# XiangpengHao/pq-vector

Measured on AMD Instinct MI355X. Metric: topk_queries_per_s_k10, higher is better.
Workload: dtype f32

## Files before the change

### pq-vector_amd/csrc/api.cpp

```cpp
#include "../../include/pqv.h"

#include <hip/hip_runtime.h>
#include <time.h>
#include <unistd.h>

#include <algorithm>
#include <atomic>
#include <functional>
#include <system_error>
#include <thread>
#include <cmath>
#include <chrono>
#include <cstdio>
#include <cstdlib>
#include <cstring>
#include <condition_variable>
#include <memory>
#include <mutex>
#include <new>
#include <string>
#include <type_traits>
#include <unordered_map>
#include <unordered_set>
#include <vector>
// ... 344 lines not shown
    mutable bool i8_residual = true;
    mutable DevBuf d_center, d_list_scale, d_list_half, d_list_radius;
    mutable DevBuf d_row_n2i, d_row_res;
    struct Opts {
        int rerank_mode = 0;
        int tile_filter = 1;
        int filter_variant = 0;
        uint32_t cand_cap = 0;
        int screen_f16 = 1;
        int screen_i8 = 1;
        uint32_t seed_rows = 0;
        uint32_t wide_rows = 0;
        uint32_t tile_rows = 0;
        int running_thr = 1;
        int defer = 1;
        int quad_xcd = -1;
        int single_bucket = 1;
        int seed_refine = 1;
        int item_grid = 1;
        int chunk_major = 1;
        int wide_waves = 0;
        int probe_rows = 1;
        int probe_screen = 1;
        uint32_t quad_width = 0;
        uint32_t min_blocks = 0;
        int pair_prune = 1;
        int i8_form = 0;
        int xcd_items = 1;
        int pf96 = 1;
        int drain_min = 0;
        int fork_wide = 0;
        int wide_quads = 1;
        uint32_t wide_quad_rows = 0;
        int list_once = 0;
    };
    mutable Opts opt;
    uint32_t n_files = 0;
    std::vector<uint32_t> seg_off;
    std::vector<uint64_t> row_base;
    uint32_t seg_max_kc = 0;
    bool rr_cap = false;
    DevBuf d_seg_off, d_seg_off64;
    mutable pqv_counters_t counters{};
    mutable bool timing = false;
    mutable std::vector<hipEvent_t> ev;
    mutable std::unique_ptr<pqv_corpus> cos_corpus;
// ... 2574 lines not shown
namespace {

void opts_from_env(pqv_searcher::Opts &o) {
    auto num = [](const char *name, long long dflt) { const char *e = std::getenv(name); return e && *e ? std::strtoll(e, nullptr, 10) : dflt; };
    if (const char *m = std::getenv("PQV_RERANK_MODE")) o.rerank_mode = !std::strcmp(m, "stream") ? 1 : !std::strcmp(m, "tile") ? 2 : 0;
    o.tile_filter = static_cast<int>(std::min<long long>(2, std::max<long long>(0, num("PQV_TILE_FILTER", o.tile_filter))));
    o.filter_variant = static_cast<int>(num("PQV_FILTER_VARIANT", o.filter_variant));
    o.cand_cap = static_cast<uint32_t>(std::max<long long>(0, num("PQV_CAND_CAP", o.cand_cap)));
    o.screen_f16 = num("PQV_SCREEN_F16", o.screen_f16) != 0;
    o.screen_i8 = static_cast<int>(num("PQV_SCREEN_I8", o.screen_i8));
    o.seed_rows = static_cast<uint32_t>(num("PQV_SEED_ROWS", o.seed_rows));
    o.wide_rows = static_cast<uint32_t>(num("PQV_WIDE_ROWS", o.wide_rows));
    o.tile_rows = static_cast<uint32_t>(num("PQV_TILE_ROWS", o.tile_rows));
    o.running_thr = num("PQV_RUNNING_THR", o.running_thr) != 0;
    o.defer = static_cast<int>(num("PQV_DEFER", o.defer));
    o.quad_xcd = static_cast<int>(num("PQV_QUAD_XCD", o.quad_xcd));
    o.wide_waves = static_cast<int>(num("PQV_WIDE_WAVES", o.wide_waves));
    o.item_grid = static_cast<int>(num("PQV_ITEM_GRID", o.item_grid));
    o.chunk_major = static_cast<int>(num("PQV_CHUNK_MAJOR", o.chunk_major));
    o.seed_refine = static_cast<int>(num("PQV_SEED_REFINE", o.seed_refine));
    o.single_bucket = static_cast<int>(num("PQV_SINGLE_BUCKET", o.single_bucket));
    o.probe_rows = static_cast<int>(num("PQV_PROBE_ROWS", o.probe_rows));
    o.probe_screen = static_cast<int>(num("PQV_PROBE_SCREEN", o.probe_screen));
    o.quad_width = static_cast<uint32_t>(num("PQV_QUAD_WIDTH", o.quad_width));
    o.min_blocks = static_cast<uint32_t>(num("PQV_MIN_BLOCKS", o.min_blocks));
    o.wide_quads = static_cast<int>(num("PQV_WIDE_QUADS", o.wide_quads));
    o.fork_wide = static_cast<int>(num("PQV_FORK_WIDE", o.fork_wide));
    o.drain_min = static_cast<int>(num("PQV_DRAIN_MIN", o.drain_min));
    o.pf96 = static_cast<int>(num("PQV_PF96", o.pf96));
    o.xcd_items = static_cast<int>(num("PQV_XCD_ITEMS", o.xcd_items));
    o.wide_quad_rows = static_cast<uint32_t>(num("PQV_WIDE_QUAD_ROWS", o.wide_quad_rows));
    o.list_once = static_cast<int>(num("PQV_LIST_ONCE", o.list_once));
    o.pair_prune = static_cast<int>(num("PQV_PAIR_PRUNE", o.pair_prune));
    o.i8_form = static_cast<int>(num("PQV_I8_FORM", o.i8_form));
}

bool wide_rows_nt(const pqv_searcher *s) {
    if (!s->h_wide_stats.p) return true;
    const volatile uint32_t *h = s->h_wide_stats.as<uint32_t>();
    const uint32_t total = h[0], lone = h[1];
    return total == 0 || static_cast<uint64_t>(lone) * 4 >= static_cast<uint64_t>(total) * 3;
}

bool prefer_regular(const pqv_searcher *s) {
    if (!s->h_wide_stats.p) return false;
    const volatile uint32_t *h = s->h_wide_stats.as<uint32_t>();
// ... 547 lines not shown
    end.assign(clusters.size(), 0);
    uint64_t fb = 0;
    j = 0;
    for (uint32_t f = 0; f < F; ++f) {
        const uint32_t kf = std::min<uint32_t>(nprobe, s->seg_off[f + 1] - s->seg_off[f]);
        for (uint32_t i = 0; i < kf && j < clusters.size(); ++i, ++j) end[j] = fb + quota[f];
        fb += cnt[f];
    }
}

void stream_split(uint64_t max_len, uint64_t pairs, uint32_t &rows_per_block, uint32_t &blocks_per_list) {
    const uint64_t bpl = std::max<uint64_t>(1, std::min<uint64_t>((8192 + pairs - 1) / pairs, (max_len + 255) / 256));
    const uint64_t rpb = ((max_len + bpl - 1) / bpl + 255) / 256 * 256;
    rows_per_block = static_cast<uint32_t>(rpb);
    blocks_per_list = static_cast<uint32_t>((max_len + rpb - 1) / rpb);
}

struct TopkPlan {
    uint32_t np;
    uint32_t probe_bpl;
    uint32_t probe_kpart;
    bool probe_rows;
    bool probe_screen;
    uint32_t rr_rows_per_block, rr_bpl;
    uint32_t n_part_probe, n_part_rr;
    bool tile;
    uint32_t max_groups;
    bool filter;
    uint32_t seed_rows, filter_bpl;
    bool f16;
    bool i8;
    bool quad;
    uint32_t filter_rows_per_block, max_quads, quad_width;
    uint32_t block_waves;
    uint32_t slots_per_pair;
    uint32_t wide_width;
    uint32_t wide_rows_per_block, wide_bpl;
    bool list_once;
};

static uint32_t cand_cap_for(const pqv_searcher *s, uint32_t k) {
    return std::max<uint32_t>(s->opt.cand_cap ? s->opt.cand_cap : (k > 32 ? 8192u : 2048u), k);
}
static bool defer_on(const pqv_searcher *s, uint32_t nq, uint32_t k, const TopkPlan &p) {
    if (s->opt.defer == 0) return false;
    if (k > 64) return true;
    const uint64_t mean_len = s->n / std::max<uint32_t>(1, s->n_clusters);
    if (s->opt.defer != 2 && mean_len > 1536 && prefer_regular(s)) return false;
    return nq >= 8 && p.i8 && p.block_waves == 4 && p.quad_width == 96 && s->sdim >= 512 && (s->opt.defer == 2 || mean_len <= 3072);
}
static bool defer_route(const pqv_searcher *s, uint32_t nq, uint32_t k, const TopkPlan &p) {
    return defer_on(s, nq, k, p) && cand_cap_for(s, k) <= 8192;
}
static bool seed_refine_on(const pqv_searcher *s, uint32_t nq, uint32_t k) {
    (void)nq;
    return s->opt.seed_refine && (!s->d_row_of || s->images_only) && (s->sdim % 32) == 0 && k <= 16 && (s->opt.seed_refine > 1 || s->sdim >= 256);
}
TopkPlan plan_topk(const pqv_searcher *s, uint32_t nq, uint32_t nprobe, uint32_t k = 1, int metric = 0, bool exact_stream = false) {
    TopkPlan p{};
    const pqv_searcher::Opts &o = s->opt;
    if (metric == PQV_DOT) exact_stream = true;
    p.np = probe_count(s, nprobe);
    p.probe_bpl = (s->n_clusters + 255) / 256;
    p.n_part_probe = p.probe_bpl * pqv::waves_per_block();
    p.probe_rows = s->opt.probe_rows && s->kc_pad != 0 && (nq >= 8 || s->opt.probe_rows > 1) &&
                   static_cast<uint64_t>(nq) * s->kc_pad * 12 <= (2ull << 30);
    if (metric == PQV_DOT) p.probe_rows = false;
    p.probe_screen = p.probe_rows && s->ps.ok && o.probe_screen && !s->n_files && p.np >= 1 && p.np <= s->n_clusters / 4 &&
                     (o.probe_screen > 1 || (nq >= 128 && s->n_clusters >= 256));
    p.probe_kpart = p.probe_rows ? 64u : p.np;
    if (s->n_files && !p.probe_rows) {
        p.probe_bpl = (s->seg_max_kc + 255) / 256;
        p.n_part_probe = s->n_files * p.probe_bpl * pqv::waves_per_block();
        p.probe_kpart = std::min<uint32_t>(nprobe, s->seg_max_kc);
    }
    const uint64_t max_len = std::max<uint64_t>(1, s->max_list_len);
    const uint64_t pairs = std::max<uint64_t>(1, static_cast<uint64_t>(nq) * p.np);
    p.tile = metric == PQV_L2SQ_REF4 && k <= 256 && pairs >= 4ull * s->n_clusters;
    const uint64_t mean_len = s->n / std::max<uint32_t>(1, s->n_clusters);
    const bool wide_ok = o.filter_variant == 0 && wide_path_possible(s);
    const bool wide_any_batch = metric == PQV_L2SQ_REF4 && o.tile_filter && k <= 128 && wide_ok && mean_len >= 192;
    if (wide_any_batch) p.tile = true;
    if (o.rerank_mode == 1) p.tile = false;
    if (o.rerank_mode == 2) p.tile = metric == PQV_L2SQ_REF4 && k <= 256;
    if (exact_stream) p.tile = false;
    if (p.tile) {
        const uint64_t est_groups = std::max<uint64_t>(1, pairs / pqv::TILE_QB);
        const uint64_t tile_rows = o.tile_rows ? o.tile_rows : 1536;
        uint64_t rpb = std::min<uint64_t>(tile_rows, (max_len + 255) / 256 * 256);
        while (rpb > 256 && est_groups * ((max_len + rpb - 1) / rpb) < 2048) rpb -= 256;
        p.rr_rows_per_block = static_cast<uint32_t>(rpb);
        p.seed_rows = o.seed_rows ? std::max<uint32_t>(64, o.seed_rows / 64 * 64)
// ... 113 lines not shown
    return PQV_OK;
}

int enqueue_probe(const pqv_searcher *s, Scratch &sc, const TopkPlan &p, const float *d_queries, uint32_t nq, uint32_t nprobe,
                  uint64_t max_candidates, const pqv::MergeArgs &pm, uint32_t *zero_u32, uint32_t zero_n, hipStream_t stream,
                  int metric = PQV_L2SQ_REF4) {
    using namespace pqv;
    uint64_t *keys = const_cast<uint64_t *>(pm.part_keys);
    uint32_t *vals = const_cast<uint32_t *>(pm.part_vals);
    if (p.probe_screen) {
        const pqv_searcher::ProbeScreen &ps = s->ps;
        HIP_TRY(sc.s_ps_q16.ensure(static_cast<size_t>(nq) * ps.dim_p * sizeof(uint16_t)));
        HIP_TRY(sc.s_ps_qn2.ensure(static_cast<size_t>(nq) * sizeof(float)));
        HIP_TRY(sc.s_ps_score.ensure(static_cast<size_t>(nq) * s->kc_pad * sizeof(float)));
        HIP_TRY(launch_center_normalize_f16(d_queries, s->d_ps_mu.as<float>(), nq, nq, s->dim, ps.dim_p, sc.s_ps_qn2.as<float>(), sc.s_ps_q16.p, stream));
        ProbeScreenArgs pr{};
        pr.q16 = sc.s_ps_q16.as<uint16_t>(); pr.c16 = s->d_ps_c16.as<uint16_t>(); pr.qn2 = sc.s_ps_qn2.as<float>(); pr.cn2 = s->d_ps_cn2.as<float>();
        pr.score = sc.s_ps_score.as<float>(); pr.queries = d_queries; pr.centroids = s->d_centroids.as<float>();
        pr.nq = nq; pr.kc = s->n_clusters; pr.kc_pad = s->kc_pad; pr.dim = s->dim; pr.dim_p = ps.dim_p; pr.np = p.np;
        pr.inv_cs = ps.inv_cs; pr.fn = ps.fn; pr.e1 = ps.e1; pr.e2s = ps.e2s; pr.kS = ps.kS; pr.lo_f = ps.lo_f; pr.hi_f = ps.hi_f;
        pr.part_keys = keys; pr.part_vals = vals;
        pr.zero_u32 = zero_u32; pr.zero_n = zero_n;
        pr.stats = s->d_ps_stats.as<unsigned long long>();
        HIP_TRY(launch_probe_screen(pr, stream));
        s->counters.kernel_launches += 2;
    } else if (p.probe_rows) {
        ProbeRowsArgs pr{};
        pr.cent_t = s->d_cent_t.as<float4>(); pr.queries = d_queries;
        pr.nq = nq; pr.kc = s->n_clusters; pr.kc_pad = s->kc_pad; pr.dim = s->dim;
        pr.part_keys = keys; pr.part_vals = vals;
        pr.zero_u32 = zero_u32; pr.zero_n = zero_n;
        HIP_TRY(launch_probe_rows(pr, stream));
    } else {
        StreamArgs pa{};
        pa.mat = s->d_centroids.as<float>();
        if (s->n_files) {
            HIP_TRY(launch_seg_probe_fill(s->d_seg_off.as<uint32_t>(), s->n_files, nq, sc.s_probe.as<uint32_t>(), sc.s_cand_base.as<uint64_t>(), stream));
            pa.list_off = s->d_seg_off64.as<uint64_t>(); pa.probe = sc.s_probe.as<uint32_t>(); pa.cand_base = sc.s_cand_base.as<uint64_t>();
            pa.nprobe = s->n_files;
        } else {
            pa.single_begin = 0; pa.single_end = s->n_clusters;
            pa.nprobe = 1;
        }
        pa.queries = d_queries; pa.nq = nq; pa.dim = s->dim; pa.k = p.probe_kpart;
        pa.rows_per_block = 256; pa.blocks_per_list = p.probe_bpl;
        pa.max_pos = ~0ull; pa.metric = PQV_L2SQ_REF4;
        pa.part_keys = keys; pa.part_vals = vals;
        pa.zero_u32 = zero_u32; pa.zero_n = zero_n;
// ... 2022 lines not shown
    else if (n == "filter_variant") o.filter_variant = static_cast<int>(value);
    else if (n == "cand_cap") o.cand_cap = static_cast<uint32_t>(std::max<int64_t>(0, value));
    else if (n == "screen_f16") o.screen_f16 = value != 0;
    else if (n == "screen_i8") o.screen_i8 = static_cast<int>(value);
    else if (n == "seed_rows") o.seed_rows = static_cast<uint32_t>(std::max<int64_t>(0, value));
    else if (n == "wide_rows") o.wide_rows = static_cast<uint32_t>(std::max<int64_t>(0, value));
    else if (n == "tile_rows") o.tile_rows = static_cast<uint32_t>(std::max<int64_t>(0, value));
    else if (n == "running_thr") o.running_thr = value != 0;
    else if (n == "defer") o.defer = static_cast<int>(value);
    else if (n == "quad_xcd") o.quad_xcd = static_cast<int>(value);
    else if (n == "wide_waves") o.wide_waves = static_cast<int>(value);
    else if (n == "single_bucket") o.single_bucket = static_cast<int>(value);
    else if (n == "seed_refine") o.seed_refine = static_cast<int>(value);
    else if (n == "item_grid") o.item_grid = static_cast<int>(value);
    else if (n == "chunk_major") o.chunk_major = value != 0;
    else if (n == "probe_rows") o.probe_rows = static_cast<int>(value);
    else if (n == "probe_screen") {
        o.probe_screen = static_cast<int>(value);
        if (value != 0 && !s->ps.tried && s->kc_pad != 0 && !s->n_files) {
            const hipError_t e = probe_screen_images(s);
            if (e != hipSuccess) return fail(e == hipErrorOutOfMemory ? PQV_ERR_OOM : PQV_ERR_HIP, std::string("probe_screen_images: ") + hipGetErrorString(e));
        }
    }
    else if (n == "quad_width") o.quad_width = static_cast<uint32_t>(std::max<int64_t>(0, value));
    else if (n == "min_blocks") o.min_blocks = static_cast<uint32_t>(std::max<int64_t>(0, value));
    else if (n == "pair_prune") o.pair_prune = value != 0;
    else if (n == "wide_quads") o.wide_quads = value <= 0 ? 0 : value >= 2 ? 2 : 1;
    else if (n == "fork_wide") o.fork_wide = value <= 0 ? 0 : value >= 2 ? 2 : 1;
    else if (n == "pf96") o.pf96 = value <= 0 ? 0 : value >= 2 ? 2 : 1;
    else if (n == "drain_min") o.drain_min = static_cast<int>(std::max<int64_t>(0, std::min<int64_t>(64, value)));
    else if (n == "xcd_items") o.xcd_items = static_cast<int>(std::max<int64_t>(0, std::min<int64_t>(3, value)));
    else if (n == "wide_quad_rows") o.wide_quad_rows = static_cast<uint32_t>(std::max<int64_t>(0, value));
    else if (n == "list_once") o.list_once = static_cast<int>(value);
    else if (n == "i8_form") {
        o.i8_form = static_cast<int>(std::min<int64_t>(2, std::max<int64_t>(0, value)));
        (void)hipSetDevice(s->device);
        (void)hipDeviceSynchronize();
        s->d_mat_blk_op[2].release();
    }
    else return fail(PQV_ERR_INVALID, "unknown searcher option: " + n);
    if (s->cos) return pqv_searcher_set_option_impl(s->cos.get(), name, value);
    return PQV_OK;
}
extern "C" int pqv_searcher_set_option(pqv_searcher *s, const char *name, int64_t value) {
    return guard([&] { return pqv_searcher_set_option_impl(s, name, value); });
}
// ... 77 lines not shown
        const bool qlds = !rt.q_global;
        const bool pf = p.f16 && s->sdim <= 128 && p.block_waves == 4 && p.quad_width != 96;
        const int op = rt.operand;
        const int seed_ng = p.i8 ? (64ull * s->sdim <= 49152 ? 4 : 2) : p.f16 ? ((64ull * s->sdim * 2 <= 32768 && p.quad_width % 64 == 0) ? 4 : 2) : static_cast<int>(p.quad_width / 16);
        const bool defp = S == 1 && rt.deferred;
        std::snprintf(kn, sizeof kn, " | kernels: wide_filter_kernel<%u, %u, %d, %s, %d, %s, %s, 4, %s>; wide_seed_kernel<%d, %s, %d, %d>; seed_select_kernel<%d>@%u",
                      p.quad_width / 16, p.block_waves, S, qlds ? "true" : "false", op, pf ? "true" : "false",
                      ((p.i8 && p.block_waves == 4 && p.quad_width == 64 && std::max<uint32_t>(1, nq) <= 64u) || p.wide_width) ? "true" : "false",
                      defp ? "true" : "false", seed_ng, qlds ? "true" : "false", op, rt.seed_tail ? 12 : 1, S,
                      std::max<uint32_t>(1, nq) * (seed_refine_on(s, std::max<uint32_t>(1, nq), k) ? 256u : 64u));
        if (p.wide_width) {
            const size_t l = std::strlen(kn);
            if (p.list_once) std::snprintf(kn + l, sizeof kn - l, "; list_filter_kernel<%u, %d>", s->sdim / 64, S);
            else
            std::snprintf(kn + l, sizeof kn - l, "; wide_filter_kernel<%u, 8, %d, true, 2, false, %s, 2, %s>", p.wide_width / 16, S, wide_rows_nt(s) ? "true" : "false",
                          defp ? "true" : "false");
        }
    }
    if (metric == PQV_DOT) {
        const bool al = (s->sdim % 4) == 0;
        std::snprintf(kn, sizeof kn, " | kernels: dot_stream_kernel<%d, %d, 0, %s, 0>; dot_merge_kernel<%d>",
                      (al && (s->sdim / 4) % 64 == 0) ? 64 : 32, k <= 64 ? 1 : k <= 256 ? 4 : 16, al ? "true" : "false", k <= 64 ? 1 : k <= 256 ? 4 : 16);
    }
    std::snprintf(buf, len, "%s%s; centroid probe: %s%s", tb, t, p.probe_screen ? "probe_screen_kernel + probe_resolve_kernel (f16 contraction, probe_rows_kernel's exact chains for the contenders)"
                  : p.probe_rows ? "probe_rows_kernel (a lane per centroid)" : metric == PQV_DOT ? "dot_stream_kernel" : "stream_kernel", kn);
    return PQV_OK;
}
extern "C" int pqv_searcher_describe(const pqv_searcher *s, uint32_t nq, uint32_t k, uint32_t nprobe, int metric,
                                     char *buf, size_t len) {
    return guard([&] { return pqv_searcher_describe_impl(s, nq, k, nprobe, metric, buf, len); });
}

static int pqv_searcher_footprint_impl(const pqv_searcher *s, uint64_t *row_order_bytes, uint64_t *ivf_rows_bytes,
                                       uint64_t *blocked_bytes, uint64_t *other_bytes) {
    if (!s) return fail(PQV_ERR_INVALID, "searcher must not be NULL");
    std::lock_guard<std::mutex> lock(s->mu);
    if (row_order_bytes) *row_order_bytes = s->corpus && s->corpus->d_rows ? s->corpus->capacity * s->corpus->dim * sizeof(float) : 0;
    if (ivf_rows_bytes) *ivf_rows_bytes = s->d_mat_ivf.p ? s->d_mat_ivf.bytes : 0;
    if (blocked_bytes) *blocked_bytes = (s->d_mat_blk_op[0].p ? s->d_mat_blk_op[0].bytes : 0) + (s->d_mat_blk_op[1].p ? s->d_mat_blk_op[1].bytes : 0) +
                                        (s->d_mat_blk_op[2].p ? s->d_mat_blk_op[2].bytes : 0);
    uint64_t other = s->d_centroids.bytes + s->d_cent_t.bytes + s->d_ps_mu.bytes + s->d_ps_c16.bytes + s->d_ps_cn2.bytes + s->d_ps_stats.bytes + s->d_list_off.bytes + s->d_ids.bytes + s->d_stats.bytes + s->d_row_norm2.bytes + s->d_blk_off.bytes +
                     s->d_center.bytes + s->d_list_scale.bytes + s->d_list_half.bytes + s->d_list_radius.bytes + s->d_row_n2i.bytes + s->d_row_res.bytes;
    for (const Scratch &l : s->lanes)
        for (const DevBuf *b : l.bufs()) other += b->p ? b->bytes : 0;
    if (other_bytes) *other_bytes = other;
    if (s->cos) {
        uint64_t f[4] = {0, 0, 0, 0};
// ... 738 lines not shown
```

### pq-vector_amd/csrc/kernels.h

```cpp
#pragma once
#include <hip/hip_runtime.h>
#include <stdint.h>

namespace pqv {

constexpr uint64_t KEY_EMPTY = ~0ull;

enum StreamMode : int {
    STREAM_TOPK   = 0,
    STREAM_DIST   = 1,
    STREAM_MINUPD = 2,
    STREAM_RANGE  = 3,
};

struct StreamArgs {
    const float    *mat;
    const uint32_t *row_of;
    const uint64_t *list_off;
    const uint32_t *probe;
    const uint64_t *cand_base;
    uint64_t        single_begin, single_end;
    const float    *queries;
    uint32_t        nq, nprobe, dim, k;
    uint32_t        rows_per_block;
// ... 202 lines not shown
    uint32_t       *zero_u32;
    uint32_t        zero_n;
};
hipError_t launch_probe_rows(const ProbeRowsArgs &a, hipStream_t s);
struct ProbeScreenArgs {
    const uint16_t *q16;
    const uint16_t *c16;
    const float    *qn2;
    const float    *cn2;
    float          *score;
    const float    *queries;
    const float    *centroids;
    uint32_t        nq, kc, kc_pad, dim, dim_p, np;
    float           inv_cs;
    float           fn;
    float           e1, e2s, kS;
    float           lo_f, hi_f;
    uint64_t       *part_keys;
    uint32_t       *part_vals;
    uint32_t       *zero_u32;
    uint32_t        zero_n;
    unsigned long long *stats;
};
hipError_t launch_probe_screen(const ProbeScreenArgs &a, hipStream_t s);
struct MergeArgs;
struct PairQuantArgs;
hipError_t launch_probe_single(const ProbeRowsArgs &pr, const MergeArgs &a, uint32_t *ticket, const PairQuantArgs *quant, hipStream_t s);
hipError_t launch_transpose_rows4(const float *rows, uint32_t kc, uint32_t kc_pad, uint32_t dim, void *out, hipStream_t s);

struct PairQuantArgs {
    const float    *queries;
    const uint32_t *probe;
    const float    *center;
    const float    *scale;
    const float    *half;
    const float    *radius;
    uint32_t        n_pairs, nprobe, dim;
    int8_t         *q_i8;
    int            *q_n2i;
    float          *q_res, *q_resu, *pair_lb;
};

struct MergeArgs {
    const uint64_t *part_keys;
    const uint32_t *part_vals;
    uint32_t        nq, n_part, k_part, k;
    const uint32_t *ids;
    uint32_t       *row_idx;
// ... 459 lines not shown
```

### pq-vector_amd/csrc/kernels_probe.hip

```cpp
#include "stream_walk.hpp"

namespace pqv {

template <int CG, int S, int MODE, bool SEQ, bool ALIGNED>
__global__ __launch_bounds__(256) void stream_kernel(const StreamArgs a) {
    if (a.zero_u32 && blockIdx.x == 0 && blockIdx.y == 0) {
        for (uint32_t i = blockIdx.z * 256 + threadIdx.x; i < a.zero_n; i += gridDim.z * 256) a.zero_u32[i] = 0u;
    }
    __shared__ float lds_all[4 * tile_words<CG, SEQ>()];
    const int lane = threadIdx.x & 63;
    const int wave = threadIdx.x >> 6;
    float *lds = lds_all + wave * tile_words<CG, SEQ>();

    const uint32_t q = blockIdx.z, j = blockIdx.y + (MODE == STREAM_RANGE ? a.j0 : 0u);
    const WalkRange w = walk_range<false>(a, q, j, wave);
    const float *qv = a.queries + (uint64_t)q * a.dim;

    WaveTopk<S> tk;
    if constexpr (MODE == STREAM_TOPK) tk.init();

    for (uint64_t t0 = w.r0; t0 < w.r1; t0 += 64) {
        const uint32_t nvalid = (w.r1 - t0 < 64) ? (uint32_t)(w.r1 - t0) : 64u;
        const uint32_t lrow = (uint32_t)lane < nvalid ? (uint32_t)lane : nvalid - 1;
        const uint32_t my_srow = storage_row(a, w.lbeg + t0 + lrow);
// ... 168 lines not shown
        a.q_resu[p] = (bad || !(ru < INFINITY)) ? INFINITY : ru;
        const float cmargin = (float)(a.dim + 16) * 2.384185791015625e-07f;
        if (a.probe) {
            const float lbd = sqrtf(v2) * 0.99998f - a.radius[c];
            const float lb = lbd > 0.0f ? lbd * lbd * (1.0f - 2.0f * cmargin) * 0.99999f : 0.0f;
            a.pair_lb[p] = (bad || !(lb < INFINITY)) ? 0.0f : lb;
        }
    }
}
__global__ __launch_bounds__(256) void quantize_pairs_i8_kernel(const PairQuantArgs a) {
    const uint32_t p = blockIdx.x * 4u + (threadIdx.x >> 6);
    if (p < a.n_pairs) quantize_pair_i8_wave(a, p, (int)(threadIdx.x & 63));
}
hipError_t launch_quantize_pairs_i8(const float *queries, const uint32_t *probe, const float *center, const float *scale, const float *half,
                                    const float *radius, uint32_t n_pairs, uint32_t nprobe, uint32_t dim, void *q_i8, int *q_n2i,
                                    float *q_res, float *q_resu, float *pair_lb, hipStream_t s) {
    if (n_pairs == 0) return hipSuccess;
    if (dim % 4 || nprobe == 0 || (probe && !pair_lb)) return hipErrorInvalidValue;
    PairQuantArgs a{queries, probe, center, scale, half, radius, n_pairs, nprobe, dim, static_cast<int8_t *>(q_i8), q_n2i, q_res, q_resu, pair_lb};
    hipLaunchKernelGGL(quantize_pairs_i8_kernel, dim3((n_pairs + 3) / 4), dim3(256), 0, s, a);
    return hipGetLastError();
}

__device__ __forceinline__ void probe_merge_helpers(const MergeArgs &a, uint32_t q) {
    if (a.preset_keys) {
        uint64_t *pk = a.preset_keys + (uint64_t)q * a.preset_n;
        uint32_t *pv = a.preset_vals + (uint64_t)q * a.preset_n;
        for (uint32_t i = threadIdx.x - 64; i < a.preset_n; i += blockDim.x - 64) { pk[i] = KEY_EMPTY; pv[i] = 0xFFFFFFFFu; }
    }
    if (a.preset_flags) {
        uint32_t *pf = reinterpret_cast<uint32_t *>(a.preset_flags + (uint64_t)q * a.preset_flag_n);
        for (uint32_t i = threadIdx.x - 64; i < a.preset_flag_n / 4; i += blockDim.x - 64) pf[i] = 0u;
    }
}
__device__ __forceinline__ void probe_query_norms(const MergeArgs &a, uint32_t q, int lane) {
    if (a.qnorm_out || a.qmax_out) {
        float acc = 0.0f, m = 0.0f;
        const float *qp = a.queries + (uint64_t)q * a.dim;
        if ((a.dim % 4u) == 0u) {
            for (uint32_t d0 = (uint32_t)lane * 4u; d0 < a.dim; d0 += 2048u) {
                float4 v[8];
#pragma unroll
                for (int u = 0; u < 8; ++u) {
                    const uint32_t d = d0 + 256u * (uint32_t)u;
                    v[u] = d < a.dim ? *reinterpret_cast<const float4 *>(qp + d) : make_float4(0.f, 0.f, 0.f, 0.f);
                }
#pragma unroll
                for (int u = 0; u < 8; ++u) {
                    acc += v[u].x * v[u].x; acc += v[u].y * v[u].y; acc += v[u].z * v[u].z; acc += v[u].w * v[u].w;
                    m = fmaxf(fmaxf(m, fmaxf(fabsf(v[u].x), fabsf(v[u].y))), fmaxf(fabsf(v[u].z), fabsf(v[u].w)));
                }
            }
        } else {
            for (uint32_t d = lane; d < a.dim; d += 64) { const float v = qp[d]; acc += v * v; m = fmaxf(m, fabsf(v)); }
        }
#pragma unroll
        for (int off = 32; off > 0; off >>= 1) { acc += __shfl_down(acc, off, 64); m = fmaxf(m, __shfl_down(m, off, 64)); }
        if (lane == 0 && a.qnorm_out) a.qnorm_out[q] = acc;
        if (lane == 0 && a.qmax_out) a.qmax_out[q] = m;
    }
}
template <int S>
__device__ __forceinline__ void probe_merge_tail(const MergeArgs &a, uint32_t q, int lane, WaveTopk<S> &tk, bool norms = true) {
    uint64_t carry = 0;
#pragma unroll
    for (int s = 0; s < S; ++s) {
        const uint32_t e = s * 64 + lane;
        const bool have = e < a.k && tk.key[s] != KEY_EMPTY;
        const uint32_t c = have ? tk.val[s] : 0;
        const uint64_t len = have ? (a.list_off[c + 1] - a.list_off[c]) : 0;
        uint64_t incl = len;
#pragma unroll
        for (int off = 1; off < 64; off <<= 1) {
            const uint32_t lo = (uint32_t)__shfl_up((int)(uint32_t)incl, off, 64);
            const uint32_t hi = (uint32_t)__shfl_up((int)(uint32_t)(incl >> 32), off, 64);
            const uint64_t o = ((uint64_t)hi << 32) | lo;
            if (lane >= off) incl += o;
        }
        if (e < a.k) {
            a.probe[(uint64_t)q * a.k + e] = c;
            a.cand_base[(uint64_t)q * a.k + e] = carry + incl - len;
            if (a.hist && have && !a.sq_quads) atomicAdd(&a.hist[(uint64_t)(q % HIST_REPLICAS) * a.hist_stride + c], 1u);
        }
        if (a.sq_quads && s == 0) {
            const uint32_t nch = (have && a.sq_item_rows) ? (uint32_t)((len + a.sq_item_rows - 1) / a.sq_item_rows) : 0u;
            uint32_t ii = nch;
#pragma unroll
            for (int off = 1; off < 64; off <<= 1) {
                const uint32_t o = (uint32_t)__shfl_up((int)ii, off, 64);
                if (lane >= off) ii += o;
            }
            const uint32_t first = ii - nch;
            if (have) {
                a.sq_quads[e] = make_uint4(c, e, 1u, first);
                a.sq_pairs[e] = e;
                for (uint32_t t = 0; t < nch && first + t < a.sq_max_items; ++t) a.sq_item_quad[first + t] = e;
            }
            const uint32_t nqd = (uint32_t)__popcll(__ballot(have));
            const uint32_t nit = readlane_u32(ii, 63);
            if (lane == 0) {
                *a.sq_n_quads = nqd;
                if (a.sq_n_items) *a.sq_n_items = nit < a.sq_max_items ? nit : a.sq_max_items;
            }
        }
        carry += readlane_u64(incl, 63);
    }
    if (a.n_cand && lane == 0) a.n_cand[q] = carry;
    if (a.stats && lane == 0) {
#ifdef PQV_PROFILE_PHASES
        unsigned long long *st = a.stats;
#else
        unsigned long long *st = a.stats + 8 + 16 * (q % STATS_SLOTS);
#endif
        atomicAdd(&st[2], (unsigned long long)carry);
        atomicAdd(&st[3], (unsigned long long)(carry < a.max_pos ? carry : a.max_pos));
    }
    if (a.gthr_init && lane == 0) a.gthr_init[q] = ~0ull;
    if (norms) probe_query_norms(a, q, lane);
}

template <int NB>
__device__ __forceinline__ void resolve_exact(const MergeArgs &a, uint32_t q, const uint16_t *band, uint32_t m, uint64_t *ck, const uint32_t *cv,
                                              int lane, int wave, uint32_t lg, float *cl = nullptr ) {
    const uint32_t Gx = a.dim >> 2;
    const uint32_t L = 1u << lg, per_wave = 64u >> lg;
    const uint32_t pl = (uint32_t)lane >> lg, pj = (uint32_t)lane & (L - 1u);
    const uint32_t first = (uint32_t)lane & ~(L - 1u);
    const float4 *qg = reinterpret_cast<const float4 *>(a.queries + (uint64_t)q * a.dim);
    for (uint32_t p0 = (uint32_t)wave * per_wave; p0 < m; p0 += 4u * per_wave) {
        const uint32_t pi = p0 + pl;
        const bool valid = pi < m;
        const uint32_t idx = band[valid ? pi : p0];
        const float *x = a.mat + (uint64_t)cv[idx] * a.dim;
        float sum = 0.0f;
        for (uint32_t g0 = 0; g0 < Gx; g0 += NB * L) {
            const uint32_t g = g0 + NB * pj;
            float4 xv[NB], qv[NB];
#pragma unroll
            for (int u = 0; u < NB; ++u) {
                const uint32_t gu = g + u < Gx ? g + u : Gx - 1;
                xv[u] = load4<true>(x + gu * 4); qv[u] = qg[gu];
            }
// ... 901 lines not shown
```

### pq-vector_amd/csrc/kernels_probe_screen.hip

```cpp
#include "device_common.hpp"

namespace pqv {

__global__ __launch_bounds__(256, 2) void probe_screen_kernel(const ProbeScreenArgs a) {
    if (a.zero_u32 && blockIdx.x == 0) {
        for (uint32_t i = blockIdx.y * 256 + threadIdx.x; i < a.zero_n; i += gridDim.y * 256) a.zero_u32[i] = 0u;
    }
    __shared__ float4 lds[4096];
    const int lane = threadIdx.x & 63, wave = __builtin_amdgcn_readfirstlane(threadIdx.x >> 6);
    const int l31 = lane & 31, lk = lane >> 5;
    float4 *const As = lds + wave * 1024, *const Bs = As + 512;
    auto sw = [](int r) { return ((r >> 1) & 1) | (((r >> 2) & 3) << 1); };
    const uint32_t q0 = blockIdx.y * 64u, c0 = blockIdx.x * 64u;
    const int ld_r = lane >> 3, ld_ch = lane & 7;
    const uint32_t rowb = a.dim_p / 8u;
    const float4 *const qb = reinterpret_cast<const float4 *>(a.q16) + (uint64_t)q0 * rowb + ld_ch;
    const float4 *const cb = reinterpret_cast<const float4 *>(a.c16) + (uint64_t)(c0 + ld_r) * rowb + ld_ch;
    uint32_t qo[8];
#pragma unroll
    for (int h = 0; h < 8; ++h) {
        const uint32_t qr = q0 + ld_r + 8 * h < a.nq ? q0 + ld_r + 8 * h : a.nq - 1;
        qo[h] = (qr - q0) * rowb;
    }
    const uint32_t nk = a.dim_p / 64u;
// ... 45 lines not shown
    }
}

struct ProbeBound { float lb, ub; };
__device__ __forceinline__ ProbeBound probe_bound(const ProbeScreenArgs &a, float an2, float an_ub, float bn2, float s) {
    const float bn_ub = sqrtf(bn2) * a.fn;
    const float est = s * (sqrtf(an2) * 0.00390625f) * a.inv_cs;
    const float S = an2 + bn2;
    const float mid = S - 2.0f * est;
    const float E = (a.kS * S + 2.0f * an_ub * (bn_ub * a.e1 + a.e2s)) * 1.00001f + 1.0e-33f;
    ProbeBound r;
    const float lo = mid - E, hi = mid + E;
    const bool finite = fabsf(S) < INFINITY && fabsf(est) < INFINITY && fabsf(mid) < INFINITY && E < INFINITY &&
                        fabsf(lo) < INFINITY && hi < 3.0e38f;
    r.lb = finite ? fmaxf(lo, 0.0f) * a.lo_f : 0.0f;
    r.ub = finite ? fmaxf(hi, 0.0f) * a.hi_f + 1.0e-33f : INFINITY;
    return r;
}

constexpr uint32_t PR_CAP = 2048;
constexpr uint32_t PR_GS = 192;
constexpr uint32_t PR_TW = PR_GS + 4;
constexpr uint32_t PR_R = 32;

__global__ __launch_bounds__(256) void probe_resolve_kernel(const ProbeScreenArgs a) {
    __shared__ uint32_t s_hist[256];
    __shared__ uint32_t s_sel[4];
    __shared__ uint32_t s_list[PR_CAP];
    __shared__ __attribute__((aligned(16))) float s_term[PR_R * PR_TW];
    const uint32_t q = blockIdx.x;
    const int lane = threadIdx.x & 63, wave = threadIdx.x >> 6;
    const float an2 = a.qn2[q];
    const float an_ub = sqrtf(an2) * a.fn;
    const float *sc = a.score + (uint64_t)q * a.kc_pad;
    uint64_t *pk = a.part_keys + (uint64_t)q * a.kc_pad;
    uint32_t *pv = a.part_vals + (uint64_t)q * a.kc_pad;
    bool all = !(an2 < INFINITY);
    float Tf = INFINITY;
    const bool parked = 2u * a.kc <= PR_R * PR_TW;
    float *s_ub = s_term, *s_lb = s_term + a.kc;
    auto bound = [&](uint32_t c) {
        ProbeBound b = probe_bound(a, an2, an_ub, a.cn2[c], sc[c]);
        if (!(b.ub < INFINITY)) b.ub = INFINITY;
        return b;
    };
    auto ub_of = [&](uint32_t c) { return parked ? s_ub[c] : bound(c).ub; };
    if (!all) {
        if (threadIdx.x == 0) { s_sel[2] = 0x7F800000u; s_sel[3] = 0u; }
        __syncthreads();
        uint32_t mn = 0x7F800000u, mx = 0u;
        for (uint32_t c = threadIdx.x; c < a.kc; c += 256) {
// ... 24 lines not shown
            uint32_t tm = 0u;
            for (uint32_t c = threadIdx.x; c < a.kc; c += 256)
                if (key_of(c) <= Tk) { const uint32_t u = __float_as_uint(ub_of(c)); tm = u > tm ? u : tm; }
#pragma unroll
            for (int off = 32; off > 0; off >>= 1) { const uint32_t o = (uint32_t)__shfl_xor((int)tm, off, 64); tm = o > tm ? o : tm; }
            if (lane == 0) atomicMax(&s_sel[3], tm);
        }
        __syncthreads();
        Tf = __uint_as_float(s_sel[3]);
        all = !(Tf < INFINITY);
    }
    __syncthreads();
    if (threadIdx.x == 0) s_sel[2] = 0u;
    __syncthreads();
    for (uint32_t c = threadIdx.x; c < a.kc_pad; c += 256) {
        bool keep = false;
        if (c < a.kc && !all) {
            const float lb = parked ? s_lb[c] : bound(c).lb;
            keep = !(lb > Tf);
        }
        if (keep) {
            const uint32_t slot = atomicAdd(&s_sel[2], 1u);
            if (slot < PR_CAP) s_list[slot] = c;
        } else {
            pk[c] = KEY_EMPTY; pv[c] = 0xFFFFFFFFu;
        }
    }
    __syncthreads();
    uint32_t m = s_sel[2];
    if (all || m > PR_CAP) { all = true; m = a.kc; }
    if (a.stats && threadIdx.x == 0) {
        atomicAdd(&a.stats[0], 1ull);
        atomicAdd(&a.stats[1], (unsigned long long)m);
        if (all) atomicAdd(&a.stats[2], 1ull);
    }
    const uint32_t G = a.dim >> 2;
    const float4 *qg = reinterpret_cast<const float4 *>(a.queries + (uint64_t)q * a.dim);
    for (uint32_t p0 = 0; p0 < m; p0 += PR_R) {
        float run = 0.0f;
        for (uint32_t gs0 = 0; gs0 < G; gs0 += PR_GS) {
            float4 qv[3];
#pragma unroll
            for (int j = 0; j < 3; ++j) {
                const uint32_t g = gs0 + (uint32_t)lane + 64u * (uint32_t)j;
                qv[j] = qg[g < G ? g : G - 1];
            }
#pragma unroll
            for (int half = 0; half < 2; ++half) {
                float4 xv[4][3];
#pragma unroll
                for (int i = 0; i < 4; ++i) {
                    const uint32_t pi = p0 + 4u * (uint32_t)(half * 4 + i) + (uint32_t)wave;
                    if (pi < m) {
// ... 17 lines not shown
                        float t = d0 * d0 + d1 * d1;
                        t = t + d2 * d2;
                        t = t + d3 * d3;
                        s_term[((uint32_t)wave * 8u + (uint32_t)(half * 4 + i)) * PR_TW + (uint32_t)lane + 64u * (uint32_t)j] = t;
                    }
            }
            __syncthreads();
            if (lane < 8) {
                const uint32_t n = G - gs0 < PR_GS ? G - gs0 : PR_GS;
                const float *row = s_term + ((uint32_t)wave * 8u + (uint32_t)lane) * PR_TW;
                uint32_t g = 0;
#pragma unroll 4
                for (; g + 4 <= n; g += 4) {
                    const float4 t = *reinterpret_cast<const float4 *>(row + g);
                    run = run + t.x; run = run + t.y; run = run + t.z; run = run + t.w;
                }
                for (; g < n; ++g) run = run + row[g];
            }
            __syncthreads();
        }
        if (lane < 8 && p0 + 4u * (uint32_t)lane + (uint32_t)wave < m) {
            const uint32_t li = p0 + 4u * (uint32_t)lane + (uint32_t)wave;
            const uint32_t c = all ? li : s_list[li];
            pk[c] = ((uint64_t)__float_as_uint(run) << 32) | c;
            pv[c] = c;
        }
    }
}

hipError_t launch_probe_screen(const ProbeScreenArgs &a, hipStream_t s) {
    if (a.nq == 0 || a.kc == 0) return hipSuccess;
    if ((a.dim % 4) != 0 || (a.dim_p % 64) != 0 || a.dim_p < a.dim || (a.kc_pad % 256) != 0 || a.kc_pad < a.kc || a.np == 0 || a.np > a.kc)
        return hipErrorInvalidValue;
    hipLaunchKernelGGL(probe_screen_kernel, dim3(a.kc_pad / 64, (a.nq + 63) / 64), dim3(256), 0, s, a);
    hipLaunchKernelGGL(probe_resolve_kernel, dim3(a.nq), dim3(256), 0, s, a);
    return hipGetLastError();
}

}
```

Baseline: 637,800.

## Fold probe top-k merge into the probe resolve kernel

Adds a templated FOLD variant of probe_resolve_kernel that keeps surviving centroid distances in LDS, ranks them by counting, and runs the probe merge tail (probe list, candidate bases, norms) inside the same block. This removes the separate merge_kernel launch and the global writes of the full per-query key/value partition arrays. When too many contenders survive, it falls back to writing the arrays and doing a wave-level selection. The rank step is O(m^2) per block over up to 1024 entries, and the merge work now runs in one wave of each resolve block.

```diff
diff --git a/pq-vector_amd/csrc/api.cpp b/pq-vector_amd/csrc/api.cpp
--- a/pq-vector_amd/csrc/api.cpp
+++ b/pq-vector_amd/csrc/api.cpp
@@ -390,6 +390,7 @@
         int wide_waves = 0;
         int probe_rows = 1;
         int probe_screen = 1;
+        int probe_fold = 1;
         uint32_t quad_width = 0;
         uint32_t min_blocks = 0;
         int pair_prune = 1;
@@ -3010,6 +3011,7 @@
     o.single_bucket = static_cast<int>(num("PQV_SINGLE_BUCKET", o.single_bucket));
     o.probe_rows = static_cast<int>(num("PQV_PROBE_ROWS", o.probe_rows));
     o.probe_screen = static_cast<int>(num("PQV_PROBE_SCREEN", o.probe_screen));
+    o.probe_fold = static_cast<int>(num("PQV_PROBE_FOLD", o.probe_fold));
     o.quad_width = static_cast<uint32_t>(num("PQV_QUAD_WIDTH", o.quad_width));
     o.min_blocks = static_cast<uint32_t>(num("PQV_MIN_BLOCKS", o.min_blocks));
     o.wide_quads = static_cast<int>(num("PQV_WIDE_QUADS", o.wide_quads));
@@ -3603,6 +3605,7 @@
     uint32_t probe_kpart;
     bool probe_rows;
     bool probe_screen;
+    bool probe_fold;
     uint32_t rr_rows_per_block, rr_bpl;
     uint32_t n_part_probe, n_part_rr;
     bool tile;
@@ -3649,6 +3652,7 @@
     if (metric == PQV_DOT) p.probe_rows = false;
     p.probe_screen = p.probe_rows && s->ps.ok && o.probe_screen && !s->n_files && p.np >= 1 && p.np <= s->n_clusters / 4 &&
                      (o.probe_screen > 1 || (nq >= 128 && s->n_clusters >= 256));
+    p.probe_fold = p.probe_screen && o.probe_fold && p.np <= 64;
     p.probe_kpart = p.probe_rows ? 64u : p.np;
     if (s->n_files && !p.probe_rows) {
         p.probe_bpl = (s->seg_max_kc + 255) / 256;
@@ -3808,8 +3812,9 @@
         pr.part_keys = keys; pr.part_vals = vals;
         pr.zero_u32 = zero_u32; pr.zero_n = zero_n;
         pr.stats = s->d_ps_stats.as<unsigned long long>();
-        HIP_TRY(launch_probe_screen(pr, stream));
-        s->counters.kernel_launches += 2;
+        HIP_TRY(launch_probe_screen(pr, p.probe_fold ? &pm : nullptr, stream));
+        s->counters.kernel_launches += p.probe_fold ? 1 : 2;
+        if (p.probe_fold) return PQV_OK;
     } else if (p.probe_rows) {
         ProbeRowsArgs pr{};
         pr.cent_t = s->d_cent_t.as<float4>(); pr.queries = d_queries;
@@ -5878,6 +5883,7 @@
             if (e != hipSuccess) return fail(e == hipErrorOutOfMemory ? PQV_ERR_OOM : PQV_ERR_HIP, std::string("probe_screen_images: ") + hipGetErrorString(e));
         }
     }
+    else if (n == "probe_fold") o.probe_fold = value != 0;
     else if (n == "quad_width") o.quad_width = static_cast<uint32_t>(std::max<int64_t>(0, value));
     else if (n == "min_blocks") o.min_blocks = static_cast<uint32_t>(std::max<int64_t>(0, value));
     else if (n == "pair_prune") o.pair_prune = value != 0;
@@ -6001,7 +6007,9 @@
         std::snprintf(kn, sizeof kn, " | kernels: dot_stream_kernel<%d, %d, 0, %s, 0>; dot_merge_kernel<%d>",
                       (al && (s->sdim / 4) % 64 == 0) ? 64 : 32, k <= 64 ? 1 : k <= 256 ? 4 : 16, al ? "true" : "false", k <= 64 ? 1 : k <= 256 ? 4 : 16);
     }
-    std::snprintf(buf, len, "%s%s; centroid probe: %s%s", tb, t, p.probe_screen ? "probe_screen_kernel + probe_resolve_kernel (f16 contraction, probe_rows_kernel's exact chains for the contenders)"
+    std::snprintf(buf, len, "%s%s; centroid probe: %s%s", tb, t,
+                  p.probe_fold ? "probe_screen_kernel + probe_resolve_kernel (f16 contraction, probe_rows_kernel's exact chains for the contenders; probe merge folded into the resolve)"
+                  : p.probe_screen ? "probe_screen_kernel + probe_resolve_kernel (f16 contraction, probe_rows_kernel's exact chains for the contenders; probe merge: merge_kernel, its own launch)"
                   : p.probe_rows ? "probe_rows_kernel (a lane per centroid)" : metric == PQV_DOT ? "dot_stream_kernel" : "stream_kernel", kn);
     return PQV_OK;
 }
diff --git a/pq-vector_amd/csrc/kernels.h b/pq-vector_amd/csrc/kernels.h
--- a/pq-vector_amd/csrc/kernels.h
+++ b/pq-vector_amd/csrc/kernels.h
@@ -248,8 +248,8 @@
     uint32_t        zero_n;
     unsigned long long *stats;
 };
-hipError_t launch_probe_screen(const ProbeScreenArgs &a, hipStream_t s);
 struct MergeArgs;
+hipError_t launch_probe_screen(const ProbeScreenArgs &a, const MergeArgs *fold, hipStream_t s);
 struct PairQuantArgs;
 hipError_t launch_probe_single(const ProbeRowsArgs &pr, const MergeArgs &a, uint32_t *ticket, const PairQuantArgs *quant, hipStream_t s);
 hipError_t launch_transpose_rows4(const float *rows, uint32_t kc, uint32_t kc_pad, uint32_t dim, void *out, hipStream_t s);
diff --git a/pq-vector_amd/csrc/kernels_probe.hip b/pq-vector_amd/csrc/kernels_probe.hip
--- a/pq-vector_amd/csrc/kernels_probe.hip
+++ b/pq-vector_amd/csrc/kernels_probe.hip
@@ -1,4 +1,5 @@
 #include "stream_walk.hpp"
+#include "probe_merge.hpp"
 
 namespace pqv {
 
@@ -214,102 +215,6 @@
     return hipGetLastError();
 }
 
-__device__ __forceinline__ void probe_merge_helpers(const MergeArgs &a, uint32_t q) {
-    if (a.preset_keys) {
-        uint64_t *pk = a.preset_keys + (uint64_t)q * a.preset_n;
-        uint32_t *pv = a.preset_vals + (uint64_t)q * a.preset_n;
-        for (uint32_t i = threadIdx.x - 64; i < a.preset_n; i += blockDim.x - 64) { pk[i] = KEY_EMPTY; pv[i] = 0xFFFFFFFFu; }
-    }
-    if (a.preset_flags) {
-        uint32_t *pf = reinterpret_cast<uint32_t *>(a.preset_flags + (uint64_t)q * a.preset_flag_n);
-        for (uint32_t i = threadIdx.x - 64; i < a.preset_flag_n / 4; i += blockDim.x - 64) pf[i] = 0u;
-    }
-}
-__device__ __forceinline__ void probe_query_norms(const MergeArgs &a, uint32_t q, int lane) {
-    if (a.qnorm_out || a.qmax_out) {
-        float acc = 0.0f, m = 0.0f;
-        const float *qp = a.queries + (uint64_t)q * a.dim;
-        if ((a.dim % 4u) == 0u) {
-            for (uint32_t d0 = (uint32_t)lane * 4u; d0 < a.dim; d0 += 2048u) {
-                float4 v[8];
-#pragma unroll
-                for (int u = 0; u < 8; ++u) {
-                    const uint32_t d = d0 + 256u * (uint32_t)u;
-                    v[u] = d < a.dim ? *reinterpret_cast<const float4 *>(qp + d) : make_float4(0.f, 0.f, 0.f, 0.f);
-                }
-#pragma unroll
-                for (int u = 0; u < 8; ++u) {
-                    acc += v[u].x * v[u].x; acc += v[u].y * v[u].y; acc += v[u].z * v[u].z; acc += v[u].w * v[u].w;
-                    m = fmaxf(fmaxf(m, fmaxf(fabsf(v[u].x), fabsf(v[u].y))), fmaxf(fabsf(v[u].z), fabsf(v[u].w)));
-                }
-            }
-        } else {
-            for (uint32_t d = lane; d < a.dim; d += 64) { const float v = qp[d]; acc += v * v; m = fmaxf(m, fabsf(v)); }
-        }
-#pragma unroll
-        for (int off = 32; off > 0; off >>= 1) { acc += __shfl_down(acc, off, 64); m = fmaxf(m, __shfl_down(m, off, 64)); }
-        if (lane == 0 && a.qnorm_out) a.qnorm_out[q] = acc;
-        if (lane == 0 && a.qmax_out) a.qmax_out[q] = m;
-    }
-}
-template <int S>
-__device__ __forceinline__ void probe_merge_tail(const MergeArgs &a, uint32_t q, int lane, WaveTopk<S> &tk, bool norms = true) {
-    uint64_t carry = 0;
-#pragma unroll
-    for (int s = 0; s < S; ++s) {
-        const uint32_t e = s * 64 + lane;
-        const bool have = e < a.k && tk.key[s] != KEY_EMPTY;
-        const uint32_t c = have ? tk.val[s] : 0;
-        const uint64_t len = have ? (a.list_off[c + 1] - a.list_off[c]) : 0;
-        uint64_t incl = len;
-#pragma unroll
-        for (int off = 1; off < 64; off <<= 1) {
-            const uint32_t lo = (uint32_t)__shfl_up((int)(uint32_t)incl, off, 64);
-            const uint32_t hi = (uint32_t)__shfl_up((int)(uint32_t)(incl >> 32), off, 64);
-            const uint64_t o = ((uint64_t)hi << 32) | lo;
-            if (lane >= off) incl += o;
-        }
-        if (e < a.k) {
-            a.probe[(uint64_t)q * a.k + e] = c;
-            a.cand_base[(uint64_t)q * a.k + e] = carry + incl - len;
-            if (a.hist && have && !a.sq_quads) atomicAdd(&a.hist[(uint64_t)(q % HIST_REPLICAS) * a.hist_stride + c], 1u);
-        }
-        if (a.sq_quads && s == 0) {
-            const uint32_t nch = (have && a.sq_item_rows) ? (uint32_t)((len + a.sq_item_rows - 1) / a.sq_item_rows) : 0u;
-            uint32_t ii = nch;
-#pragma unroll
-            for (int off = 1; off < 64; off <<= 1) {
-                const uint32_t o = (uint32_t)__shfl_up((int)ii, off, 64);
-                if (lane >= off) ii += o;
-            }
-            const uint32_t first = ii - nch;
-            if (have) {
-                a.sq_quads[e] = make_uint4(c, e, 1u, first);
-                a.sq_pairs[e] = e;
-                for (uint32_t t = 0; t < nch && first + t < a.sq_max_items; ++t) a.sq_item_quad[first + t] = e;
-            }
-            const uint32_t nqd = (uint32_t)__popcll(__ballot(have));
-            const uint32_t nit = readlane_u32(ii, 63);
-            if (lane == 0) {
-                *a.sq_n_quads = nqd;
-                if (a.sq_n_items) *a.sq_n_items = nit < a.sq_max_items ? nit : a.sq_max_items;
-            }
-        }
-        carry += readlane_u64(incl, 63);
-    }
-    if (a.n_cand && lane == 0) a.n_cand[q] = carry;
-    if (a.stats && lane == 0) {
-#ifdef PQV_PROFILE_PHASES
-        unsigned long long *st = a.stats;
-#else
-        unsigned long long *st = a.stats + 8 + 16 * (q % STATS_SLOTS);
-#endif
-        atomicAdd(&st[2], (unsigned long long)carry);
-        atomicAdd(&st[3], (unsigned long long)(carry < a.max_pos ? carry : a.max_pos));
-    }
-    if (a.gthr_init && lane == 0) a.gthr_init[q] = ~0ull;
-    if (norms) probe_query_norms(a, q, lane);
-}
 
 template <int NB>
 __device__ __forceinline__ void resolve_exact(const MergeArgs &a, uint32_t q, const uint16_t *band, uint32_t m, uint64_t *ck, const uint32_t *cv,
diff --git a/pq-vector_amd/csrc/kernels_probe_screen.hip b/pq-vector_amd/csrc/kernels_probe_screen.hip
--- a/pq-vector_amd/csrc/kernels_probe_screen.hip
+++ b/pq-vector_amd/csrc/kernels_probe_screen.hip
@@ -1,4 +1,5 @@
 #include "device_common.hpp"
+#include "probe_merge.hpp"
 
 namespace pqv {
 
@@ -91,11 +92,14 @@
 constexpr uint32_t PR_GS = 192;
 constexpr uint32_t PR_TW = PR_GS + 4;
 constexpr uint32_t PR_R = 32;
-
-__global__ __launch_bounds__(256) void probe_resolve_kernel(const ProbeScreenArgs a) {
-    __shared__ uint32_t s_hist[256];
+constexpr uint32_t PR_FOLD = 1024;
+
+template <bool FOLD>
+__global__ __launch_bounds__(256) void probe_resolve_kernel(const ProbeScreenArgs a, const MergeArgs ma) {
+    __shared__ __attribute__((aligned(8))) uint32_t s_hist[256];
     __shared__ uint32_t s_sel[4];
     __shared__ uint32_t s_list[PR_CAP];
+    __shared__ uint32_t s_dist[FOLD ? PR_FOLD : 1];
     __shared__ __attribute__((aligned(16))) float s_term[PR_R * PR_TW];
     const uint32_t q = blockIdx.x;
     const int lane = threadIdx.x & 63, wave = threadIdx.x >> 6;
@@ -166,13 +170,18 @@
         if (keep) {
             const uint32_t slot = atomicAdd(&s_sel[2], 1u);
             if (slot < PR_CAP) s_list[slot] = c;
-        } else {
+        } else if (!FOLD) {
             pk[c] = KEY_EMPTY; pv[c] = 0xFFFFFFFFu;
         }
     }
     __syncthreads();
     uint32_t m = s_sel[2];
     if (all || m > PR_CAP) { all = true; m = a.kc; }
+    const bool in_lds = FOLD && !all && m <= PR_FOLD;
+    if (FOLD && !in_lds) {
+        for (uint32_t c = threadIdx.x; c < a.kc_pad; c += 256) { pk[c] = KEY_EMPTY; pv[c] = 0xFFFFFFFFu; }
+        __syncthreads();
+    }
     if (a.stats && threadIdx.x == 0) {
         atomicAdd(&a.stats[0], 1ull);
         atomicAdd(&a.stats[1], (unsigned long long)m);
@@ -236,18 +245,47 @@
         if (lane < 8 && p0 + 4u * (uint32_t)lane + (uint32_t)wave < m) {
             const uint32_t li = p0 + 4u * (uint32_t)lane + (uint32_t)wave;
             const uint32_t c = all ? li : s_list[li];
-            pk[c] = ((uint64_t)__float_as_uint(run) << 32) | c;
-            pv[c] = c;
-        }
-    }
-}
-
-hipError_t launch_probe_screen(const ProbeScreenArgs &a, hipStream_t s) {
+            if (in_lds) {
+                s_dist[li] = __float_as_uint(run);
+            } else {
+                pk[c] = ((uint64_t)__float_as_uint(run) << 32) | c;
+                pv[c] = c;
+            }
+        }
+    }
+    if constexpr (FOLD) {
+        uint64_t *s_out = reinterpret_cast<uint64_t *>(s_hist);
+        __syncthreads();
+        if (in_lds) {
+            for (uint32_t e = threadIdx.x; e < m; e += 256) {
+                const uint64_t key = ((uint64_t)s_dist[e] << 32) | s_list[e];
+                uint32_t rank = 0;
+                for (uint32_t j = 0; j < m; ++j) rank += (((uint64_t)s_dist[j] << 32) | s_list[j]) < key ? 1u : 0u;
+                if (rank < ma.k) s_out[rank] = key;
+            }
+            __syncthreads();
+        }
+        if (wave != 0) { probe_merge_helpers(ma, q); return; }
+        WaveTopk<1> tk;
+        tk.init();
+        if (in_lds) {
+            if ((uint32_t)lane < (m < ma.k ? m : ma.k)) { tk.key[0] = s_out[lane]; tk.val[0] = (uint32_t)tk.key[0]; }
+        } else {
+            probe_select_lists(pk, pv, a.kc_pad, ma.k, lane, tk);
+        }
+        probe_merge_tail<1>(ma, q, lane, tk);
+    }
+}
+
+hipError_t launch_probe_screen(const ProbeScreenArgs &a, const MergeArgs *fold, hipStream_t s) {
     if (a.nq == 0 || a.kc == 0) return hipSuccess;
+    if (fold && (fold->k != a.np || a.np > 64 || fold->nq != a.nq || (uint64_t)fold->n_part * fold->k_part != a.kc_pad ||
+                 fold->part_keys != a.part_keys || fold->part_vals != a.part_vals)) return hipErrorInvalidValue;
     if ((a.dim % 4) != 0 || (a.dim_p % 64) != 0 || a.dim_p < a.dim || (a.kc_pad % 256) != 0 || a.kc_pad < a.kc || a.np == 0 || a.np > a.kc)
         return hipErrorInvalidValue;
     hipLaunchKernelGGL(probe_screen_kernel, dim3(a.kc_pad / 64, (a.nq + 63) / 64), dim3(256), 0, s, a);
-    hipLaunchKernelGGL(probe_resolve_kernel, dim3(a.nq), dim3(256), 0, s, a);
+    if (fold) hipLaunchKernelGGL(probe_resolve_kernel<true>, dim3(a.nq), dim3(256), 0, s, a, *fold);
+    else hipLaunchKernelGGL(probe_resolve_kernel<false>, dim3(a.nq), dim3(256), 0, s, a, MergeArgs{});
     return hipGetLastError();
 }
 
diff --git a/pq-vector_amd/csrc/probe_merge.hpp b/pq-vector_amd/csrc/probe_merge.hpp
--- /dev/null
+++ b/pq-vector_amd/csrc/probe_merge.hpp
@@ -0,0 +1,122 @@
+#pragma once
+#include "device_common.hpp"
+
+namespace pqv {
+
+__device__ __forceinline__ void probe_merge_helpers(const MergeArgs &a, uint32_t q) {
+    if (a.preset_keys) {
+        uint64_t *pk = a.preset_keys + (uint64_t)q * a.preset_n;
+        uint32_t *pv = a.preset_vals + (uint64_t)q * a.preset_n;
+        for (uint32_t i = threadIdx.x - 64; i < a.preset_n; i += blockDim.x - 64) { pk[i] = KEY_EMPTY; pv[i] = 0xFFFFFFFFu; }
+    }
+    if (a.preset_flags) {
+        uint32_t *pf = reinterpret_cast<uint32_t *>(a.preset_flags + (uint64_t)q * a.preset_flag_n);
+        for (uint32_t i = threadIdx.x - 64; i < a.preset_flag_n / 4; i += blockDim.x - 64) pf[i] = 0u;
+    }
+}
+__device__ __forceinline__ void probe_query_norms(const MergeArgs &a, uint32_t q, int lane) {
+    if (a.qnorm_out || a.qmax_out) {
+        float acc = 0.0f, m = 0.0f;
+        const float *qp = a.queries + (uint64_t)q * a.dim;
+        if ((a.dim % 4u) == 0u) {
+            for (uint32_t d0 = (uint32_t)lane * 4u; d0 < a.dim; d0 += 2048u) {
+                float4 v[8];
+#pragma unroll
+                for (int u = 0; u < 8; ++u) {
+                    const uint32_t d = d0 + 256u * (uint32_t)u;
+                    v[u] = d < a.dim ? *reinterpret_cast<const float4 *>(qp + d) : make_float4(0.f, 0.f, 0.f, 0.f);
+                }
+#pragma unroll
+                for (int u = 0; u < 8; ++u) {
+                    acc += v[u].x * v[u].x; acc += v[u].y * v[u].y; acc += v[u].z * v[u].z; acc += v[u].w * v[u].w;
+                    m = fmaxf(fmaxf(m, fmaxf(fabsf(v[u].x), fabsf(v[u].y))), fmaxf(fabsf(v[u].z), fabsf(v[u].w)));
+                }
+            }
+        } else {
+            for (uint32_t d = lane; d < a.dim; d += 64) { const float v = qp[d]; acc += v * v; m = fmaxf(m, fabsf(v)); }
+        }
+#pragma unroll
+        for (int off = 32; off > 0; off >>= 1) { acc += __shfl_down(acc, off, 64); m = fmaxf(m, __shfl_down(m, off, 64)); }
+        if (lane == 0 && a.qnorm_out) a.qnorm_out[q] = acc;
+        if (lane == 0 && a.qmax_out) a.qmax_out[q] = m;
+    }
+}
+template <int S>
+__device__ __forceinline__ void probe_merge_tail(const MergeArgs &a, uint32_t q, int lane, WaveTopk<S> &tk, bool norms = true) {
+    uint64_t carry = 0;
+#pragma unroll
+    for (int s = 0; s < S; ++s) {
+        const uint32_t e = s * 64 + lane;
+        const bool have = e < a.k && tk.key[s] != KEY_EMPTY;
+        const uint32_t c = have ? tk.val[s] : 0;
+        const uint64_t len = have ? (a.list_off[c + 1] - a.list_off[c]) : 0;
+        uint64_t incl = len;
+#pragma unroll
+        for (int off = 1; off < 64; off <<= 1) {
+            const uint32_t lo = (uint32_t)__shfl_up((int)(uint32_t)incl, off, 64);
+            const uint32_t hi = (uint32_t)__shfl_up((int)(uint32_t)(incl >> 32), off, 64);
+            const uint64_t o = ((uint64_t)hi << 32) | lo;
+            if (lane >= off) incl += o;
+        }
+        if (e < a.k) {
+            a.probe[(uint64_t)q * a.k + e] = c;
+            a.cand_base[(uint64_t)q * a.k + e] = carry + incl - len;
+            if (a.hist && have && !a.sq_quads) atomicAdd(&a.hist[(uint64_t)(q % HIST_REPLICAS) * a.hist_stride + c], 1u);
+        }
+        if (a.sq_quads && s == 0) {
+            const uint32_t nch = (have && a.sq_item_rows) ? (uint32_t)((len + a.sq_item_rows - 1) / a.sq_item_rows) : 0u;
+            uint32_t ii = nch;
+#pragma unroll
+            for (int off = 1; off < 64; off <<= 1) {
+                const uint32_t o = (uint32_t)__shfl_up((int)ii, off, 64);
+                if (lane >= off) ii += o;
+            }
+            const uint32_t first = ii - nch;
+            if (have) {
+                a.sq_quads[e] = make_uint4(c, e, 1u, first);
+                a.sq_pairs[e] = e;
+                for (uint32_t t = 0; t < nch && first + t < a.sq_max_items; ++t) a.sq_item_quad[first + t] = e;
+            }
+            const uint32_t nqd = (uint32_t)__popcll(__ballot(have));
+            const uint32_t nit = readlane_u32(ii, 63);
+            if (lane == 0) {
+                *a.sq_n_quads = nqd;
+                if (a.sq_n_items) *a.sq_n_items = nit < a.sq_max_items ? nit : a.sq_max_items;
+            }
+        }
+        carry += readlane_u64(incl, 63);
+    }
+    if (a.n_cand && lane == 0) a.n_cand[q] = carry;
+    if (a.stats && lane == 0) {
+#ifdef PQV_PROFILE_PHASES
+        unsigned long long *st = a.stats;
+#else
+        unsigned long long *st = a.stats + 8 + 16 * (q % STATS_SLOTS);
+#endif
+        atomicAdd(&st[2], (unsigned long long)carry);
+        atomicAdd(&st[3], (unsigned long long)(carry < a.max_pos ? carry : a.max_pos));
+    }
+    if (a.gthr_init && lane == 0) a.gthr_init[q] = ~0ull;
+    if (norms) probe_query_norms(a, q, lane);
+}
+
+__device__ __forceinline__ void probe_select_lists(const uint64_t *pk, const uint32_t *pv, uint64_t total, uint32_t k, int lane, WaveTopk<1> &tk) {
+    uint64_t cut = KEY_EMPTY;
+    if (total > 128) {
+        uint64_t lmin = KEY_EMPTY;
+        for (uint64_t i = lane; i < total; i += 64) { const uint64_t key = pk[i]; lmin = key < lmin ? key : lmin; }
+        uint32_t dummy = 0;
+        bitonic_sort64(lmin, dummy, lane);
+        cut = k <= 64u ? readlane_u64(lmin, (int)k - 1) : KEY_EMPTY;
+    }
+    for (uint64_t i = 0; i < total; i += 64) {
+        const uint64_t idx = i + lane;
+        uint64_t key = KEY_EMPTY;
+        uint32_t val = 0xFFFFFFFFu;
+        if (idx < total) { key = pk[idx]; val = pv[idx]; }
+        if (key > cut) key = KEY_EMPTY;
+        if (__ballot(key != KEY_EMPTY) != 0ull) tk.offer(key, val, k, lane);
+    }
+}
+
+}
```

After: 637,600, median of 2. Within noise of the previous version (-0.0%).
